# marbl/MHAP

Measured on AMD Instinct MI355X. Metric: overlaps/sec, higher is better.
Workload: dtype int64

## Files before the change

### mhap_amd/csrc/sketch_kernels.hip

```cpp
#include <cstdlib>
#include <cstring>

#include "kernels.hpp"
#include <algorithm>

namespace mhap {

constexpr int HASH_SEG = 4096;
constexpr int HASH_LUT_WORDS = 3 * 256;

void build_kmer_hash_luts(uint64_t* out) {
  const uint64_t c1 = 0x87c37b91114253d5ULL, c2 = 0x4cf5ad432745937fULL;
  const uint32_t d1 = 0xcc9e2d51U, d2 = 0x1b873593U;
  const char* acgt = "ACGT";
  for (int idx = 0; idx < 256; idx++) {
    uint64_t block = 0;
    for (int c = 0; c < 4; c++) block |= (uint64_t)(uint8_t)acgt[(idx >> (2 * c)) & 3] << (16 * c);
    uint64_t k1 = block * c1; k1 = rotl64(k1, 31); k1 *= c2;
    uint64_t k2 = block * c2; k2 = rotl64(k2, 33); k2 *= c1;
    uint32_t a = (uint32_t)block, b = (uint32_t)(block >> 32);
    a *= d1; a = rotl32(a, 15); a *= d2;
    b *= d1; b = rotl32(b, 15); b *= d2;
    out[idx] = k1; out[256 + idx] = k2; out[512 + idx] = (uint64_t)a | ((uint64_t)b << 32);
  }
// ... 1760 lines not shown
    return true;
  } else {
    const int waves_wg = (int)block.x / 64;
    const char* split_env = getenv("MHAP_MINHASH_SPLIT");
    const bool split_ok = !(split_env && atoi(split_env) == 0);
    const bool split = split_ok && waves_wg == 4 && n_weighted > 0 && n_weighted * 4 <= nblocks;
    const int nb_w = n_weighted < 0 ? nblocks : (int)std::min<int64_t>(nblocks, split ? n_weighted : (n_weighted + waves_wg - 1) / waves_wg);
    const int nb_u = n_unweighted < 0 ? nblocks : (int)std::min<int64_t>(nblocks, (n_unweighted + waves_wg - 1) / waves_wg);
    if (nb_w > 0)
      hipLaunchKernelGGL((minhash_kernel<MH_U, true, true>), dim3(nb_w), block, lds + 16, st_weighted, descs, nstrands, keys, wts, perm, info, store, luts, k, k2, H,
                         counter_w, out_rows, out_stride, out_status, status_stride, jump, jump_na, slist_w, counter + 5, qbuf_w, qcap, nullptr, split ? 1 : 0);
    char w1_path[160] = "none";
    if (nb_u > 0 && (classic || n_unweighted < 0 || waves_wg != 4)) {
      hipLaunchKernelGGL((minhash_kernel<MH_U, true, false>), dim3(nb_u), block, lds, st, descs, nstrands, keys, wts, perm, info, store, luts, k, k2, H,
                         counter_u, out_rows, out_stride, out_status, status_stride, jump, jump_na, slist, counter + 4, qbuf, qcap);
      if (witness) snprintf(w1_path, sizeof(w1_path), "classic");
    } else if (nb_u > 0) {
      W1Args a;
      a.descs = descs; a.keys = keys; a.store = store; a.luts = luts; a.info = info; a.slist = slist;
      a.n_tail = minhash_tail_strands(nblocks, n_unweighted); a.n_whole = n_unweighted - a.n_tail;
      a.rmax = max_nk > 0 ? (max_nk + 2047) >> 11 : 1;
      a.k = k; a.k2 = k2; a.H = H; a.counter = counter_u; a.stat = counter_u + 8;
      a.out_rows = out_rows; a.out_stride = out_stride; a.out_status = out_status; a.status_stride = status_stride;
      a.jump = jump_w1; a.unjump = unjump; a.jump_na = W1_JUMP_NA; a.qbuf = qbuf; a.qcap = qcap; a.merge = merge;
      {
        const char* e = getenv("MHAP_W1_STAGGER");
        const int stag = e ? atoi(e) : -1;
        a.stagger = stag >= 0 ? stag : 0;
      }
      const long long items = a.n_whole + a.n_tail * (long long)a.rmax;
      const int nb = (int)std::min<long long>(nblocks, (items + 3) / 4);
      const size_t lds1 = (size_t)H * 8 * 4 + lut_bytes;
      if (a.n_tail > 0) (void)hipMemsetAsync(merge, 0xFF, (size_t)a.n_tail * (size_t)H * 8, st);
      a.prof = nullptr;
      if (profmode) {
        static unsigned long long* dprof1 = nullptr;
        if (!dprof1) (void)hipMalloc(&dprof1, 8 * sizeof(unsigned long long));
        (void)hipMemsetAsync(dprof1, 0, 8 * sizeof(unsigned long long), st);
        a.prof = dprof1;
        static hipEvent_t pe0 = nullptr, pe1 = nullptr;
        if (!pe0) { (void)hipEventCreate(&pe0); (void)hipEventCreate(&pe1); }
        (void)hipEventRecord(pe0, st);
        if (qcap == BS_QCAP) hipLaunchKernelGGL((minhash_w1_kernel<true, true>), dim3(nb), dim3(256), lds1, st, a);
        else hipLaunchKernelGGL((minhash_w1_kernel<true, false>), dim3(nb), dim3(256), lds1, st, a);
        (void)hipEventRecord(pe1, st);
        unsigned long long hp[8];
        (void)hipMemcpyAsync(hp, dprof1, sizeof(hp), hipMemcpyDeviceToHost, st);
        (void)hipStreamSynchronize(st);
        const double tot = (double)hp[7];
        float pms = 0.f; (void)hipEventElapsedTime(&pms, pe0, pe1);
        fprintf(stderr, "[minhash w1 prof] launch %.3f ms, %d waves: mean shader clock %.0f MHz (wave-clocks / waves / time)\n", pms, nb * 4,
                pms > 0.f ? tot / ((double)nb * 4.0) / ((double)pms * 1e3) : 0.0);
        fprintf(stderr, "[minhash w1 prof] rows %llu (first-type %llu)  wave-clocks: total %.3g  key load+transpose %.1f%%  first-row slots %.1f%% (%.0f clocks/step)  "
                        "later-row slots %.1f%% (%.0f clocks/step)  drains %.1f%%  candidates/row %.0f\n", hp[4], hp[5], tot, 100.0 * hp[0] / tot, 100.0 * hp[1] / tot,
                hp[5] ? (double)hp[1] / ((double)hp[5] * H) : 0.0, 100.0 * hp[2] / tot, hp[4] > hp[5] ? (double)hp[2] / ((double)(hp[4] - hp[5]) * H) : 0.0,
                100.0 * hp[3] / tot, hp[4] ? (double)hp[6] / (double)hp[4] : 0.0);
      } else
        if (qcap == BS_QCAP) hipLaunchKernelGGL((minhash_w1_kernel<false, true>), dim3(nb), dim3(256), lds1, st, a);
        else hipLaunchKernelGGL((minhash_w1_kernel<false, false>), dim3(nb), dim3(256), lds1, st, a);
      if (a.n_tail > 0)
        hipLaunchKernelGGL(minhash_w1_finish_kernel, dim3((unsigned)((a.n_tail * (long long)H + 255) / 256)), dim3(256), 0, st, a);
      if (witness) snprintf(w1_path, sizeof(w1_path), "w1 n_whole %lld n_tail %lld rmax %d stagger %d", (long long)a.n_whole, (long long)a.n_tail, a.rmax, a.stagger);
    }
    if (witness)
      fprintf(stderr, "[minhash] strands %lld weight-1 %lld weighted %lld nblocks %d: weight-1 launch %s; weighted launch %s\n", (long long)nstrands,
              (long long)n_unweighted, (long long)n_weighted, nblocks, w1_path, nb_w > 0 ? (split ? "split" : "wave") : "none");
    return nb_w > 0;
  }
}


#ifdef MH_ORD_PROF
__device__ unsigned long long g_ord_prof[8];
#define ORD_TICK(k) do { __syncthreads(); if (threadIdx.x == 0) { const unsigned long long t_ = wall_clock64(); atomicAdd(&g_ord_prof[k], t_ - ord_t0); ord_t0 = t_; } } while (0)
#else
#define ORD_TICK(k) do { } while (0)
#endif
__device__ __forceinline__ uint32_t mm3_mul5c(uint32_t h) {
  uint32_t t;
  asm("v_lshl_add_u32 %0, %1, 2, %1" : "=v"(t) : "v"(h));
  return t + 0xe6546b64U;
}
constexpr uint32_t ORD_BUCKET_MAX = 32;
__device__ inline uint64_t okey(int32_t h, int pos) { return ((uint64_t)((uint32_t)h ^ 0x80000000u) << 32) | (uint32_t)pos; }

__global__ __launch_bounds__(ORD_THREADS) void ordered_kernel(const ReadDesc* __restrict__ descs, int64_t nstrands,
                                                              const int32_t* __restrict__ h32, const uint8_t* __restrict__ store,
                                                              const uint64_t* __restrict__ luts, int code_words, int stage_wide, int k2, int S, int cap,
                                                              int32_t* __restrict__ out_rows, int64_t out_stride,
                                                              int32_t* __restrict__ out_meta, int64_t meta_stride, int64_t first) {
  extern __shared__ __attribute__((aligned(16))) char smem[];
  uint32_t* hist = (uint32_t*)smem;
  uint32_t* part = hist + ORD_BINS;
  uint32_t* svars = part + ORD_THREADS;
  uint64_t* buf = (uint64_t*)(svars + 4);
  uint16_t* bstart = (uint16_t*)(buf + cap);
  uint32_t* stage = (uint32_t*)(bstart + ORD_BINS + 2);
  uint16_t* stage16 = (uint16_t*)stage;
  const size_t lut_off = ((size_t)ORD_BINS * 4 + (size_t)ORD_THREADS * 4 + 16 + (size_t)cap * 8 + (size_t)(ORD_BINS + 2) * 2 + (size_t)cap * (stage_wide ? 4 : 2) + 7) & ~(size_t)7;
  uint64_t* lut = (uint64_t*)(smem + lut_off);
  uint32_t* codes = (uint32_t*)(lut + 256);
  uint32_t& s_bin = svars[0]; uint32_t& s_below = svars[1]; uint32_t& s_cnt = svars[2]; uint32_t& s_fill = svars[3];
  const int64_t strand = first + (int64_t)blockIdx.x;
  if (strand >= nstrands) return;
#ifdef MH_ORD_PROF
  unsigned long long ord_t0 = wall_clock64();
#endif
  const ReadDesc rd = descs[strand >> 1];
  const int rcs = (int)(strand & 1);
  const int n = rd.length - k2 + 1;
  int32_t* meta = out_meta + strand * meta_stride;
  if (strand_skipped(rd, rcs) || n < 1) {
    if (threadIdx.x == 0) { meta[0] = 0; meta[1] = n; meta[2] = rd.length; }
    return;
  }
  const bool mat = (rd.flags & MHAP_RD_MAT) != 0;
  const int32_t* hp = h32 + rd.h2_off + (rcs ? rd.h2_stride : 0);
  if (!mat) {
    for (int i = threadIdx.x; i < 256; i += ORD_THREADS) lut[i] = luts[512 + i];
    const int ncw = (rd.length + 15) / 16 + 2;
    for (int wj = threadIdx.x; wj < ncw && wj < code_words; wj += ORD_THREADS) codes[wj] = strand_codes16(store + rd.base_off, rd.length, rcs, 16 * wj);
    __syncthreads();
  }
  ORD_TICK(0);
  auto hget = [&](int i) -> int32_t {
    if (mat) return hp[i];
    const uint32_t cw = codes_at(codes, i);
    uint32_t h = 0;
#pragma unroll
    for (int q = 0; q < 3; q++) {
      const uint64_t kk = lut[(cw >> (8 * q)) & 255u];
      h ^= (uint32_t)kk;         h = rotl32(h, 13); h = mm3_mul5c(h);
      h ^= (uint32_t)(kk >> 32); h = rotl32(h, 13); h = mm3_mul5c(h);
    }
    h ^= 24u;
    return (int32_t)fmix32(h);
  };
  const int K = S < n ? S : n;
  if (threadIdx.x == 0) { meta[0] = K; meta[1] = n; meta[2] = rd.length; }
  if (K <= 0) return;

  const double ksig = sqrt((double)K), csig = sqrt((double)cap);
  const double target = fmin((double)K + 7.0 * ksig, (double)cap - 5.0 * csig);
  if (n > cap && target >= (double)K + 3.0 * ksig) {
    const double quant = target / (double)n;
    const uint32_t cut_u = quant >= 1.0 ? 0xFFFFFFFFu : (uint32_t)(quant * 4294967296.0);
    const uint32_t cutbin = cut_u >> 21;
    for (uint32_t j = threadIdx.x; j < ORD_BINS; j += ORD_THREADS) hist[j] = 0;
    if (threadIdx.x == 0) { s_fill = 0; s_cnt = 0; }
    __syncthreads();
    const int lane = threadIdx.x & 63;
    for (int ib = 0; ib < n; ib += 8 * ORD_THREADS) {
      const int p0 = ib + 32 * (int)(threadIdx.x >> 2) + (int)(threadIdx.x & 3);
      int32_t hv[8];
      if (mat) {
#pragma unroll
        for (int u = 0; u < 8; u++) { const int i = p0 + 4 * u; hv[u] = i < n ? hp[i] : 0; }
      } else if (p0 < n) {
        const int d = p0 >> 4;
        const uint32_t sh = (uint32_t)(2 * (p0 & 15));
        const uint32_t w0 = codes[d], w1 = codes[d + 1], w2 = codes[d + 2], w3 = codes[d + 3];
        const uint32_t a[3] = {__builtin_amdgcn_alignbit(w1, w0, sh), __builtin_amdgcn_alignbit(w2, w1, sh), __builtin_amdgcn_alignbit(w3, w2, sh)};
        uint64_t g[10];
#pragma unroll
        for (int j = 0; j < 10; j++) g[j] = lut[(a[j >> 2] >> (8 * (j & 3))) & 255u];
#pragma unroll
        for (int u = 0; u < 8; u++) {
          uint32_t h = 0;
#pragma unroll
          for (int q = 0; q < 3; q++) {
            const uint64_t kk = g[u + q];
            h ^= (uint32_t)kk;         h = rotl32(h, 13); h = mm3_mul5c(h);
            h ^= (uint32_t)(kk >> 32); h = rotl32(h, 13); h = mm3_mul5c(h);
          }
          h ^= 24u;
          hv[u] = (int32_t)fmix32(h);
        }
      } else {
#pragma unroll
        for (int u = 0; u < 8; u++) hv[u] = 0;
      }
      unsigned long long bal[8];
      uint32_t total = 0;
#pragma unroll
      for (int u = 0; u < 8; u++) {
        bal[u] = __ballot(p0 + 4 * u < n && ((uint32_t)hv[u] ^ 0x80000000u) < cut_u);
        total += (uint32_t)__popcll(bal[u]);
      }
      if (total) {
        uint32_t base = 0;
        if (lane == 0) base = atomicAdd(&s_fill, total);
        base = (uint32_t)__builtin_amdgcn_readfirstlane((int)base);
#pragma unroll
        for (int u = 0; u < 8; u++) {
          if ((bal[u] >> lane) & 1ULL) {
            const uint32_t idx = base + __builtin_amdgcn_mbcnt_hi((uint32_t)(bal[u] >> 32), __builtin_amdgcn_mbcnt_lo((uint32_t)bal[u], 0u));
            if (idx < (uint32_t)cap) { if (stage_wide) stage[idx] = (uint32_t)(p0 + 4 * u); else stage16[idx] = (uint16_t)(p0 + 4 * u); }
            atomicAdd(&hist[((uint32_t)hv[u] ^ 0x80000000u) >> 21], 1u);
          }
          base += (uint32_t)__popcll(bal[u]);
        }
      }
    }
    __syncthreads();
    ORD_TICK(1);
    const uint32_t m = s_fill;
    bool ok = m >= (uint32_t)K && m <= (uint32_t)cap;
    if (ok) {
      const int per = ORD_BINS / ORD_THREADS;
      uint32_t loc = 0, mx = 0;
      for (int j = 0; j < per; j++) { const uint32_t c = hist[threadIdx.x * per + j]; loc += c; mx = c > mx ? c : mx; }
      uint32_t incl = loc;
#pragma unroll
      for (int off = 1; off < 64; off <<= 1) { const uint32_t v = __shfl_up(incl, off); if (lane >= off) incl += v; }
      if (lane == 63) part[threadIdx.x >> 6] = incl;
      if (mx > ORD_BUCKET_MAX) atomicMax(&s_cnt, mx);
      __syncthreads();
      for (unsigned w = 0; w < (threadIdx.x >> 6); w++) incl += part[w];
      uint32_t run = incl - loc;
      for (int j = 0; j < per; j++) { const uint32_t b = threadIdx.x * per + j; bstart[b] = (uint16_t)run; run += hist[b]; }
      ok = s_cnt == 0;
      __syncthreads();
    }
    ORD_TICK(2);
    if (ok) {
      for (uint32_t b = threadIdx.x; b <= cutbin; b += ORD_THREADS) hist[b] = 0;
      __syncthreads();
      for (uint32_t t0 = threadIdx.x; t0 < m; t0 += 4 * ORD_THREADS) {
        int ii[4]; uint64_t key[4]; uint32_t slot[4];
#pragma unroll
        for (int u = 0; u < 4; u++) { const uint32_t t = t0 + (uint32_t)u * ORD_THREADS; ii[u] = t < m ? (stage_wide ? (int)stage[t] : (int)stage16[t]) : 0; }
#pragma unroll
        for (int u = 0; u < 4; u++) key[u] = okey(hget(ii[u]), ii[u]);
#pragma unroll
        for (int u = 0; u < 4; u++) { const uint32_t b = (uint32_t)(key[u] >> 53); slot[u] = t0 + (uint32_t)u * ORD_THREADS < m ? (uint32_t)bstart[b] + atomicAdd(&hist[b], 1u) : 0xFFFFFFFFu; }
#pragma unroll
        for (int u = 0; u < 4; u++) if (slot[u] != 0xFFFFFFFFu) buf[slot[u]] = key[u];
      }
      __syncthreads();
      ORD_TICK(3);
      int32_t* orow = out_rows + strand * out_stride;
      for (uint32_t t0 = threadIdx.x; t0 < m; t0 += 2 * ORD_THREADS) {
        uint64_t key[2]; uint32_t s0[2], c[2], rank[2] = {0u, 0u};
#pragma unroll
        for (int u = 0; u < 2; u++) {
          const uint32_t t = t0 + (uint32_t)u * ORD_THREADS;
          key[u] = buf[t < m ? t : t0];
          const uint32_t b = (uint32_t)(key[u] >> 53);
          s0[u] = bstart[b]; c[u] = t < m ? hist[b] : 0u;
        }
        const uint32_t cmax = c[0] > c[1] ? c[0] : c[1];
        for (uint32_t q = 0; q < cmax; q += 4) {
          uint64_t o[2][4];
#pragma unroll
          for (int u = 0; u < 2; u++)
#pragma unroll
            for (int x = 0; x < 4; x++) o[u][x] = buf[s0[u] + q + (uint32_t)x < (uint32_t)cap ? s0[u] + q + (uint32_t)x : s0[u]];
#pragma unroll
          for (int u = 0; u < 2; u++)
#pragma unroll
            for (int x = 0; x < 4; x++) rank[u] += (q + (uint32_t)x < c[u] && o[u][x] < key[u]) ? 1u : 0u;
        }
#pragma unroll
        for (int u = 0; u < 2; u++) {
          const uint32_t j = s0[u] + rank[u];
          if (t0 + (uint32_t)u * ORD_THREADS < m && j < (uint32_t)K) { orow[2 * j] = (int32_t)((uint32_t)(key[u] >> 32) ^ 0x80000000u); orow[2 * j + 1] = (int32_t)(uint32_t)key[u]; }
        }
      }
      ORD_TICK(5);
#ifdef MH_ORD_PROF
      if (threadIdx.x == 0) atomicAdd(&g_ord_prof[7], 1ULL);
#endif
      return;
    }
    __syncthreads();
  }

  uint64_t bound = ~0ULL;
  bool buckets = false;
  uint32_t bk_bin = 0, bk_total = 0;
  if (threadIdx.x == 0) s_fill = 0;
  if (n > cap) {
    const int shifts[6] = {53, 42, 32, 21, 10, 0};
    const int widths[6] = {11, 11, 10, 11, 11, 10};
    uint64_t prefix = 0;
    uint64_t prefmask = 0;
    uint32_t below = 0;
    for (int lv = 0; lv < 6; lv++) {
      const int sh = shifts[lv];
      const uint32_t nb = 1u << widths[lv];
      for (uint32_t j = threadIdx.x; j < ORD_BINS; j += ORD_THREADS) hist[j] = 0;
      __syncthreads();
      for (int i0 = threadIdx.x; i0 < n; i0 += 8 * ORD_THREADS) {
        int32_t hv[8];
#pragma unroll
        for (int u = 0; u < 8; u++) { const int i = i0 + u * ORD_THREADS; hv[u] = i < n ? hget(i) : 0; }
#pragma unroll
        for (int u = 0; u < 8; u++) {
          const int i = i0 + u * ORD_THREADS;
          const uint64_t key = okey(hv[u], i);
          if (i < n && (key & prefmask) == prefix) atomicAdd(&hist[(uint32_t)(key >> sh) & (nb - 1)], 1u);
        }
      }
      __syncthreads();
      const uint32_t target = (uint32_t)(K - 1) - below;
      const int per = ORD_BINS / ORD_THREADS;
      uint32_t loc = 0;
      for (int j = 0; j < per; j++) loc += hist[threadIdx.x * per + j];
      uint32_t incl = loc;
#pragma unroll
      for (int off = 1; off < 64; off <<= 1) {
        const uint32_t v = __shfl_up(incl, off);
        if ((threadIdx.x & 63) >= (unsigned)off) incl += v;
      }
      if ((threadIdx.x & 63) == 63) part[threadIdx.x >> 6] = incl;
      __syncthreads();
      for (unsigned w = 0; w < (threadIdx.x >> 6); w++) incl += part[w];
      const uint32_t excl = incl - loc;
      if (target >= excl && target < incl) {
        uint32_t run = excl;
        for (int j = 0; j < per; j++) {
          const uint32_t c = hist[threadIdx.x * per + j];
          if (target < run + c) { s_bin = threadIdx.x * per + j; s_below = run; s_cnt = c; break; }
          run += c;
        }
      }
      __syncthreads();
      const uint32_t bin = s_bin, binbelow = s_below, bincnt = s_cnt;
      __syncthreads();
      below += binbelow;
      prefix |= (uint64_t)bin << sh;
      prefmask |= (uint64_t)(nb - 1) << sh;
      bound = prefix | (sh > 0 ? ((1ULL << sh) - 1) : 0ULL);
      if (below + bincnt <= (uint32_t)cap) {
        if (lv == 0) {
          uint32_t run = excl, mx = 0;
          for (int j = 0; j < per; j++) {
            const uint32_t b = threadIdx.x * per + j, c = hist[b];
            if (b <= bin) { bstart[b] = (uint16_t)run; mx = c > mx ? c : mx; }
            run += c;
          }
          if (mx > ORD_BUCKET_MAX) atomicMax(&s_fill, mx);
          __syncthreads();
          buckets = s_fill == 0;
          bk_bin = bin; bk_total = below + bincnt;
          __syncthreads();
          if (threadIdx.x == 0) s_fill = 0;
        }
        break;
      }
    }
  }
  if (buckets) {
    for (uint32_t b = threadIdx.x; b <= bk_bin; b += ORD_THREADS) hist[b] = 0;
    __syncthreads();
    for (int i0 = threadIdx.x; i0 < n; i0 += 8 * ORD_THREADS) {
      int32_t hv[8];
#pragma unroll
      for (int u = 0; u < 8; u++) { const int i = i0 + u * ORD_THREADS; hv[u] = i < n ? hget(i) : 0; }
#pragma unroll
      for (int u = 0; u < 8; u++) {
        const int i = i0 + u * ORD_THREADS;
        const uint64_t key = okey(hv[u], i);
        const uint32_t b = (uint32_t)(key >> 53);
        if (i < n && b <= bk_bin) buf[(uint32_t)bstart[b] + atomicAdd(&hist[b], 1u)] = key;
      }
    }
    __syncthreads();
    int32_t* orow = out_rows + strand * out_stride;
    for (uint32_t t = threadIdx.x; t < bk_total; t += ORD_THREADS) {
      const uint64_t key = buf[t];
      const uint32_t b = (uint32_t)(key >> 53), s0 = bstart[b], c = hist[b];
      uint32_t rank = 0;
      for (uint32_t q = 0; q < c; q += 4) {
        uint64_t o[4];
#pragma unroll
        for (int x = 0; x < 4; x++) o[x] = buf[s0 + q + (uint32_t)x < (uint32_t)cap ? s0 + q + (uint32_t)x : s0];
#pragma unroll
        for (int x = 0; x < 4; x++) rank += (q + (uint32_t)x < c && o[x] < key) ? 1u : 0u;
      }
      const uint32_t j = s0 + rank;
      if (j < (uint32_t)K) { orow[2 * j] = (int32_t)((uint32_t)(key >> 32) ^ 0x80000000u); orow[2 * j + 1] = (int32_t)(uint32_t)key; }
    }
    return;
  }
  __syncthreads();
  for (int i = threadIdx.x; i < n; i += ORD_THREADS) {
    const uint64_t key = okey(hget(i), i);
    if (key <= bound) { uint32_t slot = atomicAdd(&s_fill, 1u); if (slot < (uint32_t)cap) buf[slot] = key; }
  }
  __syncthreads();
  const uint32_t m = s_fill < (uint32_t)cap ? s_fill : (uint32_t)cap;
  uint32_t np2 = 1;
  while (np2 < m) np2 <<= 1;
  for (uint32_t j = m + threadIdx.x; j < np2; j += ORD_THREADS) buf[j] = ~0ULL;
  __syncthreads();
  for (uint32_t size = 2; size <= np2; size <<= 1) {
    for (uint32_t stride = size >> 1; stride > 0; stride >>= 1) {
      for (uint32_t t = threadIdx.x; t < (np2 >> 1); t += ORD_THREADS) {
        const uint32_t lo = 2 * t - (t & (stride - 1));
        const uint32_t hi = lo + stride;
        const bool up = ((lo & size) == 0);
        const uint64_t a = buf[lo], b = buf[hi];
        if ((a > b) == up) { buf[lo] = b; buf[hi] = a; }
      }
      __syncthreads();
    }
  }
  int32_t* orow = out_rows + strand * out_stride;
  for (int j = threadIdx.x; j < K; j += ORD_THREADS) {
    const uint64_t key = buf[j];
    orow[2 * j] = (int32_t)((uint32_t)(key >> 32) ^ 0x80000000u);
    orow[2 * j + 1] = (int32_t)(uint32_t)key;
  }
}

#ifndef MH_ORD_PAD
#define MH_ORD_PAD 0
#endif
size_t ordered_lds_bytes(int cap, int code_words, int stage_wide) {
  return (size_t)ORD_BINS * 4 + (size_t)ORD_THREADS * 4 + 16 + (size_t)cap * 8 + (size_t)(ORD_BINS + 2) * 2 + (size_t)cap * (stage_wide ? 4 : 2) +
         (code_words > 0 ? (size_t)256 * 8 + (size_t)code_words * 4 : 0) + 8 + MH_ORD_PAD;
}

__global__ void fix_status_kernel(int32_t* __restrict__ meta, int64_t nreads) {
  const int64_t i = (int64_t)blockIdx.x * blockDim.x + threadIdx.x;
  if (i >= nreads) return;
  const int32_t fs = meta[(2 * i) * META_W + 3];
  if (fs != 0 && meta[(2 * i + 1) * META_W + 3] == 0) meta[(2 * i + 1) * META_W + 3] = fs;
}

void launch_fix_status(hipStream_t st, int32_t* meta, int64_t nreads) {
  if (nreads <= 0) return;
  hipLaunchKernelGGL(fix_status_kernel, dim3((unsigned)((nreads + 255) / 256)), dim3(256), 0, st, meta, nreads);
}

void launch_ordered(hipStream_t st, const ReadDesc* descs, int64_t nstrands, int max_len_codes, int max_len, const int32_t* h32,
                    const uint8_t* store, const uint64_t* luts, int k2, int S, int cap, int32_t* out_rows, int64_t out_stride,
                    int32_t* out_meta, int64_t meta_stride, int64_t first, int64_t count) {
  if (count < 0 || first + count > nstrands) count = nstrands - first;
  if (nstrands <= 0 || count <= 0) return;
  const int code_words = max_len_codes > 0 ? (max_len_codes + 15) / 16 + 4 : 0;
  const int stage_wide = max_len - k2 + 1 > 65535 ? 1 : 0;
  hipLaunchKernelGGL(ordered_kernel, dim3((unsigned)count), dim3(ORD_THREADS), ordered_lds_bytes(cap, code_words, stage_wide), st, descs, nstrands, h32,
                     store, luts, code_words, stage_wide, k2, S, cap, out_rows, out_stride, out_meta, meta_stride, first);
#ifdef MH_ORD_PROF
  (void)hipStreamSynchronize(st);
  unsigned long long hp[8];
  (void)hipMemcpyFromSymbol(hp, HIP_SYMBOL(g_ord_prof), sizeof(hp));
  fprintf(stderr, "[ordered prof] cap %d lds %zu strands(one-pass) %llu  100MHz ticks/strand: stage %.1f pass1 %.1f scan %.1f fill %.1f isort %.1f out %.1f\n", cap,
          ordered_lds_bytes(cap, code_words, stage_wide), hp[7], (double)hp[0] / hp[7], (double)hp[1] / hp[7], (double)hp[2] / hp[7], (double)hp[3] / hp[7],
          (double)hp[4] / hp[7], (double)hp[5] / hp[7]);
  unsigned long long z[8] = {0, 0, 0, 0, 0, 0, 0, 0};
  (void)hipMemcpyToSymbol(HIP_SYMBOL(g_ord_prof), z, sizeof(z));
#endif
}

}
```

Baseline: 445,000.

## Process both strands of a read in one double-width ordered-sketch workgroup

The ordered kernel now launches one 512-thread workgroup per read instead of one 256-thread block per strand. Each half handles one strand from a single shared copy of the forward 2-bit codes, and the reverse complement is built on the fly with a bit-reverse trick. The histogram bin count is sized from cap with an adaptive shift, and bucket offsets are packed into the histogram words to save LDS. This cuts the duplicated code staging and per-block overhead, but adds LDS per workgroup (two buffers), which may reduce occupancy and makes the fallback path more complex.

```diff
diff --git a/mhap_amd/csrc/sketch_kernels.hip b/mhap_amd/csrc/sketch_kernels.hip
--- a/mhap_amd/csrc/sketch_kernels.hip
+++ b/mhap_amd/csrc/sketch_kernels.hip
@@ -1866,50 +1866,81 @@
   return t + 0xe6546b64U;
 }
 constexpr uint32_t ORD_BUCKET_MAX = 32;
+constexpr int ORD_WG = 2 * ORD_THREADS;
+constexpr int ORD_PADW = 4;
 __device__ inline uint64_t okey(int32_t h, int pos) { return ((uint64_t)((uint32_t)h ^ 0x80000000u) << 32) | (uint32_t)pos; }
-
-__global__ __launch_bounds__(ORD_THREADS) void ordered_kernel(const ReadDesc* __restrict__ descs, int64_t nstrands,
-                                                              const int32_t* __restrict__ h32, const uint8_t* __restrict__ store,
-                                                              const uint64_t* __restrict__ luts, int code_words, int stage_wide, int k2, int S, int cap,
-                                                              int32_t* __restrict__ out_rows, int64_t out_stride,
-                                                              int32_t* __restrict__ out_meta, int64_t meta_stride, int64_t first) {
+__device__ __forceinline__ uint32_t rc_codes16(uint32_t x) {
+  x = __builtin_bitreverse32(x);
+  return ~(((x >> 1) & 0x55555555u) | ((x & 0x55555555u) << 1));
+}
+__host__ __device__ inline int ord_bins(int cap) { return cap / 4 < 256 ? 256 : (cap / 4 > ORD_BINS ? ORD_BINS : cap / 4); }
+struct OrdLds {
+  size_t half, uni, buf, lut, codes, total;
+  __host__ __device__ OrdLds(int cap, int code_words, int stage_wide) {
+    half = ((size_t)ord_bins(cap) * 4 + (size_t)cap * (stage_wide ? 4 : 2) + 7) & ~(size_t)7;
+    const size_t exact = (size_t)ORD_BINS * 4 + (((size_t)(ORD_BINS + 2) * 2 + 7) & ~(size_t)7);
+    uni = 96;
+    buf = uni + (2 * half > exact ? 2 * half : exact);
+    lut = buf + (size_t)cap * 16;
+    codes = lut + (code_words > 0 ? (size_t)256 * 8 : 0);
+    total = codes + (code_words > 0 ? (size_t)(ORD_PADW + code_words) * 4 : 0);
+  }
+};
+
+__global__ __launch_bounds__(ORD_WG) void ordered_kernel(const ReadDesc* __restrict__ descs, int64_t nreads,
+                                                         const int32_t* __restrict__ h32, const uint8_t* __restrict__ store,
+                                                         const uint64_t* __restrict__ luts, int code_words, int stage_wide, int k2, int S, int cap,
+                                                         int32_t* __restrict__ out_rows, int64_t out_stride,
+                                                         int32_t* __restrict__ out_meta, int64_t meta_stride, int64_t first_read) {
   extern __shared__ __attribute__((aligned(16))) char smem[];
-  uint32_t* hist = (uint32_t*)smem;
-  uint32_t* part = hist + ORD_BINS;
-  uint32_t* svars = part + ORD_THREADS;
-  uint64_t* buf = (uint64_t*)(svars + 4);
-  uint16_t* bstart = (uint16_t*)(buf + cap);
-  uint32_t* stage = (uint32_t*)(bstart + ORD_BINS + 2);
-  uint16_t* stage16 = (uint16_t*)stage;
-  const size_t lut_off = ((size_t)ORD_BINS * 4 + (size_t)ORD_THREADS * 4 + 16 + (size_t)cap * 8 + (size_t)(ORD_BINS + 2) * 2 + (size_t)cap * (stage_wide ? 4 : 2) + 7) & ~(size_t)7;
-  uint64_t* lut = (uint64_t*)(smem + lut_off);
-  uint32_t* codes = (uint32_t*)(lut + 256);
-  uint32_t& s_bin = svars[0]; uint32_t& s_below = svars[1]; uint32_t& s_cnt = svars[2]; uint32_t& s_fill = svars[3];
-  const int64_t strand = first + (int64_t)blockIdx.x;
-  if (strand >= nstrands) return;
+  const OrdLds L(cap, code_words, stage_wide);
+  uint32_t* svars = (uint32_t*)smem;
+  uint32_t* part = svars + 16;
+  uint64_t* lut = (uint64_t*)(smem + L.lut);
+  uint32_t* cf = (uint32_t*)(smem + L.codes);
+  const int64_t read = first_read + (int64_t)blockIdx.x;
+  if (read >= nreads) return;
 #ifdef MH_ORD_PROF
   unsigned long long ord_t0 = wall_clock64();
 #endif
-  const ReadDesc rd = descs[strand >> 1];
-  const int rcs = (int)(strand & 1);
-  const int n = rd.length - k2 + 1;
-  int32_t* meta = out_meta + strand * meta_stride;
-  if (strand_skipped(rd, rcs) || n < 1) {
-    if (threadIdx.x == 0) { meta[0] = 0; meta[1] = n; meta[2] = rd.length; }
-    return;
-  }
+  const ReadDesc rd = descs[read];
+  const int Lr = rd.length;
+  const int n = Lr - k2 + 1;
+  const int K = S < n ? S : n;
+  const int hs = (int)(threadIdx.x >> 8);
+  const uint32_t tl = threadIdx.x & (ORD_THREADS - 1);
+  const int lane = threadIdx.x & 63;
+  const bool act0 = !strand_skipped(rd, 0) && n >= 1 && K > 0;
+  const bool act1 = !strand_skipped(rd, 1) && n >= 1 && K > 0;
+  if (tl == 0) {
+    int32_t* meta = out_meta + (2 * read + hs) * meta_stride;
+    meta[0] = (strand_skipped(rd, hs) || n < 1) ? 0 : K; meta[1] = n; meta[2] = Lr;
+  }
+  if (!act0 && !act1) return;
   const bool mat = (rd.flags & MHAP_RD_MAT) != 0;
-  const int32_t* hp = h32 + rd.h2_off + (rcs ? rd.h2_stride : 0);
   if (!mat) {
-    for (int i = threadIdx.x; i < 256; i += ORD_THREADS) lut[i] = luts[512 + i];
-    const int ncw = (rd.length + 15) / 16 + 2;
-    for (int wj = threadIdx.x; wj < ncw && wj < code_words; wj += ORD_THREADS) codes[wj] = strand_codes16(store + rd.base_off, rd.length, rcs, 16 * wj);
+    const uint32_t* W = (const uint32_t*)(store + rd.base_off);
+    const int nd = (Lr + 15) >> 4;
+    const int ncw = min(nd + 2, code_words);
+    if (threadIdx.x < 256) lut[threadIdx.x] = luts[512 + threadIdx.x];
+    if (threadIdx.x < ORD_PADW) cf[threadIdx.x] = 0u;
+    uint32_t v[2];
+#pragma unroll
+    for (int u = 0; u < 2; u++) { const int w = (int)threadIdx.x + u * ORD_WG; v[u] = w < nd ? W[w] : 0u; }
+#pragma unroll
+    for (int u = 0; u < 2; u++) { const int w = (int)threadIdx.x + u * ORD_WG; if (w < ncw) cf[ORD_PADW + w] = v[u]; }
+    for (int w = (int)threadIdx.x + 2 * ORD_WG; w < ncw; w += ORD_WG) cf[ORD_PADW + w] = w < nd ? W[w] : 0u;
     __syncthreads();
   }
   ORD_TICK(0);
-  auto hget = [&](int i) -> int32_t {
-    if (mat) return hp[i];
-    const uint32_t cw = codes_at(codes, i);
+  auto cwin = [&](int s, int p) -> uint32_t {
+    const int q = (s ? Lr - 16 - p : p) + 16 * ORD_PADW;
+    const uint32_t x = __builtin_amdgcn_alignbit(cf[(q >> 4) + 1], cf[q >> 4], (uint32_t)(2 * (q & 15)));
+    return s ? rc_codes16(x) : x;
+  };
+  auto hget = [&](int s, int i) -> int32_t {
+    if (mat) return h32[rd.h2_off + (s ? rd.h2_stride : 0) + i];
+    const uint32_t cw = cwin(s, i);
     uint32_t h = 0;
 #pragma unroll
     for (int q = 0; q < 3; q++) {
@@ -1920,118 +1951,138 @@
     h ^= 24u;
     return (int32_t)fmix32(h);
   };
-  const int K = S < n ? S : n;
-  if (threadIdx.x == 0) { meta[0] = K; meta[1] = n; meta[2] = rd.length; }
-  if (K <= 0) return;
-
+
+  bool need0 = act0, need1 = act1;
   const double ksig = sqrt((double)K), csig = sqrt((double)cap);
   const double target = fmin((double)K + 7.0 * ksig, (double)cap - 5.0 * csig);
   if (n > cap && target >= (double)K + 3.0 * ksig) {
     const double quant = target / (double)n;
     const uint32_t cut_u = quant >= 1.0 ? 0xFFFFFFFFu : (uint32_t)(quant * 4294967296.0);
-    const uint32_t cutbin = cut_u >> 21;
-    for (uint32_t j = threadIdx.x; j < ORD_BINS; j += ORD_THREADS) hist[j] = 0;
-    if (threadIdx.x == 0) { s_fill = 0; s_cnt = 0; }
-    __syncthreads();
-    const int lane = threadIdx.x & 63;
-    for (int ib = 0; ib < n; ib += 8 * ORD_THREADS) {
-      const int p0 = ib + 32 * (int)(threadIdx.x >> 2) + (int)(threadIdx.x & 3);
-      int32_t hv[8];
-      if (mat) {
-#pragma unroll
-        for (int u = 0; u < 8; u++) { const int i = p0 + 4 * u; hv[u] = i < n ? hp[i] : 0; }
-      } else if (p0 < n) {
-        const int d = p0 >> 4;
-        const uint32_t sh = (uint32_t)(2 * (p0 & 15));
-        const uint32_t w0 = codes[d], w1 = codes[d + 1], w2 = codes[d + 2], w3 = codes[d + 3];
-        const uint32_t a[3] = {__builtin_amdgcn_alignbit(w1, w0, sh), __builtin_amdgcn_alignbit(w2, w1, sh), __builtin_amdgcn_alignbit(w3, w2, sh)};
-        uint64_t g[10];
-#pragma unroll
-        for (int j = 0; j < 10; j++) g[j] = lut[(a[j >> 2] >> (8 * (j & 3))) & 255u];
+    const int nbins = ord_bins(cap);
+    const int lgb = 31 - __builtin_clz((uint32_t)nbins);
+    const int hb = cut_u ? 31 - __builtin_clz(cut_u) : -1;
+    const int bsh = hb + 1 - lgb > 0 ? hb + 1 - lgb : 0;
+    const bool act = hs ? act1 : act0;
+    uint32_t* hist = (uint32_t*)(smem + L.uni + (size_t)hs * L.half);
+    uint32_t* stage = hist + nbins;
+    uint16_t* stage16 = (uint16_t*)stage;
+    uint64_t* buf = (uint64_t*)(smem + L.buf) + (size_t)hs * cap;
+    uint32_t& s_fill = svars[hs];
+    uint32_t& s_cnt = svars[2 + hs];
+    for (uint32_t j = tl; j < (uint32_t)nbins; j += ORD_THREADS) hist[j] = 0;
+    if (tl == 0) { s_fill = 0; s_cnt = 0; }
+    __syncthreads();
+    if (act) {
+      const int32_t* hp = h32 + rd.h2_off + (hs ? rd.h2_stride : 0);
+      for (int ib = 0; ib < n; ib += 8 * ORD_THREADS) {
+        const int p0 = ib + 32 * (int)(tl >> 2) + (int)(tl & 3);
+        int32_t hv[8];
+        if (mat) {
+#pragma unroll
+          for (int u = 0; u < 8; u++) { const int i = p0 + 4 * u; hv[u] = i < n ? hp[i] : 0; }
+        } else if (p0 < n) {
+          const int q = (hs ? Lr - 48 - p0 : p0) + 16 * ORD_PADW;
+          const int d = q >> 4;
+          const uint32_t sh = (uint32_t)(2 * (q & 15));
+          const uint32_t w0 = cf[d], w1 = cf[d + 1], w2 = cf[d + 2], w3 = cf[d + 3];
+          const uint32_t b0 = __builtin_amdgcn_alignbit(w1, w0, sh), b1 = __builtin_amdgcn_alignbit(w2, w1, sh), b2 = __builtin_amdgcn_alignbit(w3, w2, sh);
+          const uint32_t a[3] = {hs ? rc_codes16(b2) : b0, hs ? rc_codes16(b1) : b1, hs ? rc_codes16(b0) : b2};
+          uint64_t g[10];
+#pragma unroll
+          for (int j = 0; j < 10; j++) g[j] = lut[(a[j >> 2] >> (8 * (j & 3))) & 255u];
+#pragma unroll
+          for (int u = 0; u < 8; u++) {
+            uint32_t h = 0;
+#pragma unroll
+            for (int qq = 0; qq < 3; qq++) {
+              const uint64_t kk = g[u + qq];
+              h ^= (uint32_t)kk;         h = rotl32(h, 13); h = mm3_mul5c(h);
+              h ^= (uint32_t)(kk >> 32); h = rotl32(h, 13); h = mm3_mul5c(h);
+            }
+            h ^= 24u;
+            hv[u] = (int32_t)fmix32(h);
+          }
+        } else {
+#pragma unroll
+          for (int u = 0; u < 8; u++) hv[u] = 0;
+        }
+        unsigned long long bal[8];
+        uint32_t total = 0;
 #pragma unroll
         for (int u = 0; u < 8; u++) {
-          uint32_t h = 0;
-#pragma unroll
-          for (int q = 0; q < 3; q++) {
-            const uint64_t kk = g[u + q];
-            h ^= (uint32_t)kk;         h = rotl32(h, 13); h = mm3_mul5c(h);
-            h ^= (uint32_t)(kk >> 32); h = rotl32(h, 13); h = mm3_mul5c(h);
+          bal[u] = __ballot(p0 + 4 * u < n && ((uint32_t)hv[u] ^ 0x80000000u) < cut_u);
+          total += (uint32_t)__popcll(bal[u]);
+        }
+        if (total) {
+          uint32_t base = 0;
+          if (lane == 0) base = atomicAdd(&s_fill, total);
+          base = (uint32_t)__builtin_amdgcn_readfirstlane((int)base);
+#pragma unroll
+          for (int u = 0; u < 8; u++) {
+            if ((bal[u] >> lane) & 1ULL) {
+              const uint32_t idx = base + __builtin_amdgcn_mbcnt_hi((uint32_t)(bal[u] >> 32), __builtin_amdgcn_mbcnt_lo((uint32_t)bal[u], 0u));
+              if (idx < (uint32_t)cap) { if (stage_wide) stage[idx] = (uint32_t)(p0 + 4 * u); else stage16[idx] = (uint16_t)(p0 + 4 * u); }
+              atomicAdd(&hist[(((uint32_t)hv[u] ^ 0x80000000u) >> bsh) & (uint32_t)(nbins - 1)], 1u);
+            }
+            base += (uint32_t)__popcll(bal[u]);
           }
-          h ^= 24u;
-          hv[u] = (int32_t)fmix32(h);
-        }
-      } else {
-#pragma unroll
-        for (int u = 0; u < 8; u++) hv[u] = 0;
-      }
-      unsigned long long bal[8];
-      uint32_t total = 0;
-#pragma unroll
-      for (int u = 0; u < 8; u++) {
-        bal[u] = __ballot(p0 + 4 * u < n && ((uint32_t)hv[u] ^ 0x80000000u) < cut_u);
-        total += (uint32_t)__popcll(bal[u]);
-      }
-      if (total) {
-        uint32_t base = 0;
-        if (lane == 0) base = atomicAdd(&s_fill, total);
-        base = (uint32_t)__builtin_amdgcn_readfirstlane((int)base);
-#pragma unroll
-        for (int u = 0; u < 8; u++) {
-          if ((bal[u] >> lane) & 1ULL) {
-            const uint32_t idx = base + __builtin_amdgcn_mbcnt_hi((uint32_t)(bal[u] >> 32), __builtin_amdgcn_mbcnt_lo((uint32_t)bal[u], 0u));
-            if (idx < (uint32_t)cap) { if (stage_wide) stage[idx] = (uint32_t)(p0 + 4 * u); else stage16[idx] = (uint16_t)(p0 + 4 * u); }
-            atomicAdd(&hist[((uint32_t)hv[u] ^ 0x80000000u) >> 21], 1u);
-          }
-          base += (uint32_t)__popcll(bal[u]);
         }
       }
     }
     __syncthreads();
     ORD_TICK(1);
     const uint32_t m = s_fill;
-    bool ok = m >= (uint32_t)K && m <= (uint32_t)cap;
+    bool ok = act && m >= (uint32_t)K && m <= (uint32_t)cap;
+    const int per = nbins / ORD_THREADS;
+    uint32_t loc = 0, incl = 0;
     if (ok) {
-      const int per = ORD_BINS / ORD_THREADS;
-      uint32_t loc = 0, mx = 0;
-      for (int j = 0; j < per; j++) { const uint32_t c = hist[threadIdx.x * per + j]; loc += c; mx = c > mx ? c : mx; }
-      uint32_t incl = loc;
+      uint32_t mx = 0;
+      for (int j = 0; j < per; j++) { const uint32_t c = hist[tl * per + j]; loc += c; mx = c > mx ? c : mx; }
+      incl = loc;
 #pragma unroll
       for (int off = 1; off < 64; off <<= 1) { const uint32_t v = __shfl_up(incl, off); if (lane >= off) incl += v; }
       if (lane == 63) part[threadIdx.x >> 6] = incl;
       if (mx > ORD_BUCKET_MAX) atomicMax(&s_cnt, mx);
-      __syncthreads();
-      for (unsigned w = 0; w < (threadIdx.x >> 6); w++) incl += part[w];
+    }
+    __syncthreads();
+    ok = ok && s_cnt == 0;
+    if (ok) {
+      for (uint32_t w = 0; w < (tl >> 6); w++) incl += part[(threadIdx.x >> 8) * 4 + w];
       uint32_t run = incl - loc;
-      for (int j = 0; j < per; j++) { const uint32_t b = threadIdx.x * per + j; bstart[b] = (uint16_t)run; run += hist[b]; }
-      ok = s_cnt == 0;
-      __syncthreads();
-    }
+      for (int j = 0; j < per; j++) { const uint32_t b = tl * per + j, c = hist[b]; hist[b] = run << 16; run += c; }
+    }
+    __syncthreads();
     ORD_TICK(2);
     if (ok) {
-      for (uint32_t b = threadIdx.x; b <= cutbin; b += ORD_THREADS) hist[b] = 0;
-      __syncthreads();
-      for (uint32_t t0 = threadIdx.x; t0 < m; t0 += 4 * ORD_THREADS) {
+      for (uint32_t t0 = tl; t0 < m; t0 += 4 * ORD_THREADS) {
         int ii[4]; uint64_t key[4]; uint32_t slot[4];
 #pragma unroll
         for (int u = 0; u < 4; u++) { const uint32_t t = t0 + (uint32_t)u * ORD_THREADS; ii[u] = t < m ? (stage_wide ? (int)stage[t] : (int)stage16[t]) : 0; }
 #pragma unroll
-        for (int u = 0; u < 4; u++) key[u] = okey(hget(ii[u]), ii[u]);
-#pragma unroll
-        for (int u = 0; u < 4; u++) { const uint32_t b = (uint32_t)(key[u] >> 53); slot[u] = t0 + (uint32_t)u * ORD_THREADS < m ? (uint32_t)bstart[b] + atomicAdd(&hist[b], 1u) : 0xFFFFFFFFu; }
+        for (int u = 0; u < 4; u++) key[u] = okey(hget(hs, ii[u]), ii[u]);
+#pragma unroll
+        for (int u = 0; u < 4; u++) {
+          const uint32_t b = (uint32_t)(key[u] >> (32 + bsh)) & (uint32_t)(nbins - 1);
+          uint32_t w = 0xFFFFFFFFu;
+          if (t0 + (uint32_t)u * ORD_THREADS < m) { w = atomicAdd(&hist[b], 1u); w = (w >> 16) + (w & 0xFFFFu); }
+          slot[u] = w;
+        }
 #pragma unroll
         for (int u = 0; u < 4; u++) if (slot[u] != 0xFFFFFFFFu) buf[slot[u]] = key[u];
       }
-      __syncthreads();
-      ORD_TICK(3);
-      int32_t* orow = out_rows + strand * out_stride;
-      for (uint32_t t0 = threadIdx.x; t0 < m; t0 += 2 * ORD_THREADS) {
+    }
+    __syncthreads();
+    ORD_TICK(3);
+    if (ok) {
+      int32_t* orow = out_rows + (2 * read + hs) * out_stride;
+      for (uint32_t t0 = tl; t0 < m; t0 += 2 * ORD_THREADS) {
         uint64_t key[2]; uint32_t s0[2], c[2], rank[2] = {0u, 0u};
 #pragma unroll
         for (int u = 0; u < 2; u++) {
           const uint32_t t = t0 + (uint32_t)u * ORD_THREADS;
           key[u] = buf[t < m ? t : t0];
-          const uint32_t b = (uint32_t)(key[u] >> 53);
-          s0[u] = bstart[b]; c[u] = t < m ? hist[b] : 0u;
+          const uint32_t hw = hist[(uint32_t)(key[u] >> (32 + bsh)) & (uint32_t)(nbins - 1)];
+          s0[u] = hw >> 16; c[u] = t < m ? (hw & 0xFFFFu) : 0u;
         }
         const uint32_t cmax = c[0] > c[1] ? c[0] : c[1];
         for (uint32_t q = 0; q < cmax; q += 4) {
@@ -2051,161 +2102,168 @@
           if (t0 + (uint32_t)u * ORD_THREADS < m && j < (uint32_t)K) { orow[2 * j] = (int32_t)((uint32_t)(key[u] >> 32) ^ 0x80000000u); orow[2 * j + 1] = (int32_t)(uint32_t)key[u]; }
         }
       }
-      ORD_TICK(5);
+    }
+    ORD_TICK(5);
 #ifdef MH_ORD_PROF
-      if (threadIdx.x == 0) atomicAdd(&g_ord_prof[7], 1ULL);
+    if (threadIdx.x == 0) atomicAdd(&g_ord_prof[7], 1ULL);
 #endif
-      return;
-    }
-    __syncthreads();
-  }
-
-  uint64_t bound = ~0ULL;
-  bool buckets = false;
-  uint32_t bk_bin = 0, bk_total = 0;
-  if (threadIdx.x == 0) s_fill = 0;
-  if (n > cap) {
-    const int shifts[6] = {53, 42, 32, 21, 10, 0};
-    const int widths[6] = {11, 11, 10, 11, 11, 10};
-    uint64_t prefix = 0;
-    uint64_t prefmask = 0;
-    uint32_t below = 0;
-    for (int lv = 0; lv < 6; lv++) {
-      const int sh = shifts[lv];
-      const uint32_t nb = 1u << widths[lv];
-      for (uint32_t j = threadIdx.x; j < ORD_BINS; j += ORD_THREADS) hist[j] = 0;
-      __syncthreads();
-      for (int i0 = threadIdx.x; i0 < n; i0 += 8 * ORD_THREADS) {
-        int32_t hv[8];
-#pragma unroll
-        for (int u = 0; u < 8; u++) { const int i = i0 + u * ORD_THREADS; hv[u] = i < n ? hget(i) : 0; }
-#pragma unroll
-        for (int u = 0; u < 8; u++) {
-          const int i = i0 + u * ORD_THREADS;
-          const uint64_t key = okey(hv[u], i);
-          if (i < n && (key & prefmask) == prefix) atomicAdd(&hist[(uint32_t)(key >> sh) & (nb - 1)], 1u);
+    const uint32_t m0 = svars[0], m1 = svars[1];
+    need0 = act0 && !(m0 >= (uint32_t)K && m0 <= (uint32_t)cap && svars[2] == 0);
+    need1 = act1 && !(m1 >= (uint32_t)K && m1 <= (uint32_t)cap && svars[3] == 0);
+    if (!need0 && !need1) return;
+    __syncthreads();
+  }
+
+  uint32_t* hist = (uint32_t*)(smem + L.uni);
+  uint16_t* bstart = (uint16_t*)(smem + L.uni + (size_t)ORD_BINS * 4);
+  uint64_t* buf = (uint64_t*)(smem + L.buf);
+  uint32_t& s_bin = svars[4]; uint32_t& s_below = svars[5]; uint32_t& s_cnt = svars[6]; uint32_t& s_fill = svars[7];
+  for (int s = 0; s < 2; s++) {
+    if (!(s ? need1 : need0)) continue;
+    uint64_t bound = ~0ULL;
+    bool buckets = false;
+    uint32_t bk_bin = 0, bk_total = 0;
+    __syncthreads();
+    if (threadIdx.x == 0) s_fill = 0;
+    if (n > cap) {
+      const int shifts[6] = {53, 42, 32, 21, 10, 0};
+      const int widths[6] = {11, 11, 10, 11, 11, 10};
+      uint64_t prefix = 0;
+      uint64_t prefmask = 0;
+      uint32_t below = 0;
+      for (int lv = 0; lv < 6; lv++) {
+        const int sh = shifts[lv];
+        const uint32_t nb = 1u << widths[lv];
+        for (uint32_t j = threadIdx.x; j < ORD_BINS; j += ORD_WG) hist[j] = 0;
+        __syncthreads();
+        for (int i0 = threadIdx.x; i0 < n; i0 += 8 * ORD_WG) {
+          int32_t hv[8];
+#pragma unroll
+          for (int u = 0; u < 8; u++) { const int i = i0 + u * ORD_WG; hv[u] = i < n ? hget(s, i) : 0; }
+#pragma unroll
+          for (int u = 0; u < 8; u++) {
+            const int i = i0 + u * ORD_WG;
+            const uint64_t key = okey(hv[u], i);
+            if (i < n && (key & prefmask) == prefix) atomicAdd(&hist[(uint32_t)(key >> sh) & (nb - 1)], 1u);
+          }
         }
-      }
-      __syncthreads();
-      const uint32_t target = (uint32_t)(K - 1) - below;
-      const int per = ORD_BINS / ORD_THREADS;
-      uint32_t loc = 0;
-      for (int j = 0; j < per; j++) loc += hist[threadIdx.x * per + j];
-      uint32_t incl = loc;
-#pragma unroll
-      for (int off = 1; off < 64; off <<= 1) {
-        const uint32_t v = __shfl_up(incl, off);
-        if ((threadIdx.x & 63) >= (unsigned)off) incl += v;
-      }
-      if ((threadIdx.x & 63) == 63) part[threadIdx.x >> 6] = incl;
-      __syncthreads();
-      for (unsigned w = 0; w < (threadIdx.x >> 6); w++) incl += part[w];
-      const uint32_t excl = incl - loc;
-      if (target >= excl && target < incl) {
-        uint32_t run = excl;
-        for (int j = 0; j < per; j++) {
-          const uint32_t c = hist[threadIdx.x * per + j];
-          if (target < run + c) { s_bin = threadIdx.x * per + j; s_below = run; s_cnt = c; break; }
-          run += c;
+        __syncthreads();
+        const uint32_t target = (uint32_t)(K - 1) - below;
+        const int per = ORD_BINS / ORD_WG;
+        uint32_t loc = 0;
+        for (int j = 0; j < per; j++) loc += hist[threadIdx.x * per + j];
+        uint32_t incl = loc;
+#pragma unroll
+        for (int off = 1; off < 64; off <<= 1) {
+          const uint32_t v = __shfl_up(incl, off);
+          if ((threadIdx.x & 63) >= (unsigned)off) incl += v;
         }
-      }
-      __syncthreads();
-      const uint32_t bin = s_bin, binbelow = s_below, bincnt = s_cnt;
-      __syncthreads();
-      below += binbelow;
-      prefix |= (uint64_t)bin << sh;
-      prefmask |= (uint64_t)(nb - 1) << sh;
-      bound = prefix | (sh > 0 ? ((1ULL << sh) - 1) : 0ULL);
-      if (below + bincnt <= (uint32_t)cap) {
-        if (lv == 0) {
-          uint32_t run = excl, mx = 0;
+        if ((threadIdx.x & 63) == 63) part[threadIdx.x >> 6] = incl;
+        __syncthreads();
+        for (unsigned w = 0; w < (threadIdx.x >> 6); w++) incl += part[w];
+        const uint32_t excl = incl - loc;
+        if (target >= excl && target < incl) {
+          uint32_t run = excl;
           for (int j = 0; j < per; j++) {
-            const uint32_t b = threadIdx.x * per + j, c = hist[b];
-            if (b <= bin) { bstart[b] = (uint16_t)run; mx = c > mx ? c : mx; }
+            const uint32_t c = hist[threadIdx.x * per + j];
+            if (target < run + c) { s_bin = threadIdx.x * per + j; s_below = run; s_cnt = c; break; }
             run += c;
           }
-          if (mx > ORD_BUCKET_MAX) atomicMax(&s_fill, mx);
-          __syncthreads();
-          buckets = s_fill == 0;
-          bk_bin = bin; bk_total = below + bincnt;
-          __syncthreads();
-          if (threadIdx.x == 0) s_fill = 0;
         }
-        break;
-      }
-    }
-  }
-  if (buckets) {
-    for (uint32_t b = threadIdx.x; b <= bk_bin; b += ORD_THREADS) hist[b] = 0;
-    __syncthreads();
-    for (int i0 = threadIdx.x; i0 < n; i0 += 8 * ORD_THREADS) {
-      int32_t hv[8];
-#pragma unroll
-      for (int u = 0; u < 8; u++) { const int i = i0 + u * ORD_THREADS; hv[u] = i < n ? hget(i) : 0; }
-#pragma unroll
-      for (int u = 0; u < 8; u++) {
-        const int i = i0 + u * ORD_THREADS;
-        const uint64_t key = okey(hv[u], i);
-        const uint32_t b = (uint32_t)(key >> 53);
-        if (i < n && b <= bk_bin) buf[(uint32_t)bstart[b] + atomicAdd(&hist[b], 1u)] = key;
-      }
-    }
-    __syncthreads();
-    int32_t* orow = out_rows + strand * out_stride;
-    for (uint32_t t = threadIdx.x; t < bk_total; t += ORD_THREADS) {
-      const uint64_t key = buf[t];
-      const uint32_t b = (uint32_t)(key >> 53), s0 = bstart[b], c = hist[b];
-      uint32_t rank = 0;
-      for (uint32_t q = 0; q < c; q += 4) {
-        uint64_t o[4];
-#pragma unroll
-        for (int x = 0; x < 4; x++) o[x] = buf[s0 + q + (uint32_t)x < (uint32_t)cap ? s0 + q + (uint32_t)x : s0];
-#pragma unroll
-        for (int x = 0; x < 4; x++) rank += (q + (uint32_t)x < c && o[x] < key) ? 1u : 0u;
-      }
-      const uint32_t j = s0 + rank;
-      if (j < (uint32_t)K) { orow[2 * j] = (int32_t)((uint32_t)(key >> 32) ^ 0x80000000u); orow[2 * j + 1] = (int32_t)(uint32_t)key; }
-    }
-    return;
-  }
-  __syncthreads();
-  for (int i = threadIdx.x; i < n; i += ORD_THREADS) {
-    const uint64_t key = okey(hget(i), i);
-    if (key <= bound) { uint32_t slot = atomicAdd(&s_fill, 1u); if (slot < (uint32_t)cap) buf[slot] = key; }
-  }
-  __syncthreads();
-  const uint32_t m = s_fill < (uint32_t)cap ? s_fill : (uint32_t)cap;
-  uint32_t np2 = 1;
-  while (np2 < m) np2 <<= 1;
-  for (uint32_t j = m + threadIdx.x; j < np2; j += ORD_THREADS) buf[j] = ~0ULL;
-  __syncthreads();
-  for (uint32_t size = 2; size <= np2; size <<= 1) {
-    for (uint32_t stride = size >> 1; stride > 0; stride >>= 1) {
-      for (uint32_t t = threadIdx.x; t < (np2 >> 1); t += ORD_THREADS) {
-        const uint32_t lo = 2 * t - (t & (stride - 1));
-        const uint32_t hi = lo + stride;
-        const bool up = ((lo & size) == 0);
-        const uint64_t a = buf[lo], b = buf[hi];
-        if ((a > b) == up) { buf[lo] = b; buf[hi] = a; }
-      }
+        __syncthreads();
+        const uint32_t bin = s_bin, binbelow = s_below, bincnt = s_cnt;
+        __syncthreads();
+        below += binbelow;
+        prefix |= (uint64_t)bin << sh;
+        prefmask |= (uint64_t)(nb - 1) << sh;
+        bound = prefix | (sh > 0 ? ((1ULL << sh) - 1) : 0ULL);
+        if (below + bincnt <= (uint32_t)cap) {
+          if (lv == 0) {
+            uint32_t run = excl, mx = 0;
+            for (int j = 0; j < per; j++) {
+              const uint32_t b = threadIdx.x * per + j, c = hist[b];
+              if (b <= bin) { bstart[b] = (uint16_t)run; mx = c > mx ? c : mx; }
+              run += c;
+            }
+            if (mx > ORD_BUCKET_MAX) atomicMax(&s_fill, mx);
+            __syncthreads();
+            buckets = s_fill == 0;
+            bk_bin = bin; bk_total = below + bincnt;
+            __syncthreads();
+            if (threadIdx.x == 0) s_fill = 0;
+          }
+          break;
+        }
+      }
+    }
+    int32_t* orow = out_rows + (2 * read + s) * out_stride;
+    if (buckets) {
+      for (uint32_t b = threadIdx.x; b <= bk_bin; b += ORD_WG) hist[b] = 0;
       __syncthreads();
-    }
-  }
-  int32_t* orow = out_rows + strand * out_stride;
-  for (int j = threadIdx.x; j < K; j += ORD_THREADS) {
-    const uint64_t key = buf[j];
-    orow[2 * j] = (int32_t)((uint32_t)(key >> 32) ^ 0x80000000u);
-    orow[2 * j + 1] = (int32_t)(uint32_t)key;
+      for (int i0 = threadIdx.x; i0 < n; i0 += 8 * ORD_WG) {
+        int32_t hv[8];
+#pragma unroll
+        for (int u = 0; u < 8; u++) { const int i = i0 + u * ORD_WG; hv[u] = i < n ? hget(s, i) : 0; }
+#pragma unroll
+        for (int u = 0; u < 8; u++) {
+          const int i = i0 + u * ORD_WG;
+          const uint64_t key = okey(hv[u], i);
+          const uint32_t b = (uint32_t)(key >> 53);
+          if (i < n && b <= bk_bin) buf[(uint32_t)bstart[b] + atomicAdd(&hist[b], 1u)] = key;
+        }
+      }
+      __syncthreads();
+      for (uint32_t t = threadIdx.x; t < bk_total; t += ORD_WG) {
+        const uint64_t key = buf[t];
+        const uint32_t b = (uint32_t)(key >> 53), s0 = bstart[b], c = hist[b];
+        uint32_t rank = 0;
+        for (uint32_t q = 0; q < c; q += 4) {
+          uint64_t o[4];
+#pragma unroll
+          for (int x = 0; x < 4; x++) o[x] = buf[s0 + q + (uint32_t)x < (uint32_t)cap ? s0 + q + (uint32_t)x : s0];
+#pragma unroll
+          for (int x = 0; x < 4; x++) rank += (q + (uint32_t)x < c && o[x] < key) ? 1u : 0u;
+        }
+        const uint32_t j = s0 + rank;
+        if (j < (uint32_t)K) { orow[2 * j] = (int32_t)((uint32_t)(key >> 32) ^ 0x80000000u); orow[2 * j + 1] = (int32_t)(uint32_t)key; }
+      }
+      continue;
+    }
+    __syncthreads();
+    for (int i = threadIdx.x; i < n; i += ORD_WG) {
+      const uint64_t key = okey(hget(s, i), i);
+      if (key <= bound) { uint32_t slot = atomicAdd(&s_fill, 1u); if (slot < (uint32_t)cap) buf[slot] = key; }
+    }
+    __syncthreads();
+    const uint32_t m = s_fill < (uint32_t)cap ? s_fill : (uint32_t)cap;
+    uint32_t np2 = 1;
+    while (np2 < m) np2 <<= 1;
+    for (uint32_t j = m + threadIdx.x; j < np2; j += ORD_WG) buf[j] = ~0ULL;
+    __syncthreads();
+    for (uint32_t size = 2; size <= np2; size <<= 1) {
+      for (uint32_t stride = size >> 1; stride > 0; stride >>= 1) {
+        for (uint32_t t = threadIdx.x; t < (np2 >> 1); t += ORD_WG) {
+          const uint32_t lo = 2 * t - (t & (stride - 1));
+          const uint32_t hi = lo + stride;
+          const bool up = ((lo & size) == 0);
+          const uint64_t a = buf[lo], b = buf[hi];
+          if ((a > b) == up) { buf[lo] = b; buf[hi] = a; }
+        }
+        __syncthreads();
+      }
+    }
+    for (int j = threadIdx.x; j < K; j += ORD_WG) {
+      const uint64_t key = buf[j];
+      orow[2 * j] = (int32_t)((uint32_t)(key >> 32) ^ 0x80000000u);
+      orow[2 * j + 1] = (int32_t)(uint32_t)key;
+    }
   }
 }
 
 #ifndef MH_ORD_PAD
 #define MH_ORD_PAD 0
 #endif
-size_t ordered_lds_bytes(int cap, int code_words, int stage_wide) {
-  return (size_t)ORD_BINS * 4 + (size_t)ORD_THREADS * 4 + 16 + (size_t)cap * 8 + (size_t)(ORD_BINS + 2) * 2 + (size_t)cap * (stage_wide ? 4 : 2) +
-         (code_words > 0 ? (size_t)256 * 8 + (size_t)code_words * 4 : 0) + 8 + MH_ORD_PAD;
-}
+size_t ordered_lds_bytes(int cap, int code_words, int stage_wide) { return OrdLds(cap, code_words, stage_wide).total + MH_ORD_PAD; }
 
 __global__ void fix_status_kernel(int32_t* __restrict__ meta, int64_t nreads) {
   const int64_t i = (int64_t)blockIdx.x * blockDim.x + threadIdx.x;
@@ -2224,15 +2282,17 @@
                     int32_t* out_meta, int64_t meta_stride, int64_t first, int64_t count) {
   if (count < 0 || first + count > nstrands) count = nstrands - first;
   if (nstrands <= 0 || count <= 0) return;
+  const int64_t nreads = nstrands / 2, r0 = first / 2, r1 = std::min<int64_t>(nreads, (first + count + 1) / 2);
+  if (r1 <= r0) return;
   const int code_words = max_len_codes > 0 ? (max_len_codes + 15) / 16 + 4 : 0;
   const int stage_wide = max_len - k2 + 1 > 65535 ? 1 : 0;
-  hipLaunchKernelGGL(ordered_kernel, dim3((unsigned)count), dim3(ORD_THREADS), ordered_lds_bytes(cap, code_words, stage_wide), st, descs, nstrands, h32,
-                     store, luts, code_words, stage_wide, k2, S, cap, out_rows, out_stride, out_meta, meta_stride, first);
+  hipLaunchKernelGGL(ordered_kernel, dim3((unsigned)(r1 - r0)), dim3(ORD_WG), ordered_lds_bytes(cap, code_words, stage_wide), st, descs, nreads, h32,
+                     store, luts, code_words, stage_wide, k2, S, cap, out_rows, out_stride, out_meta, meta_stride, r0);
 #ifdef MH_ORD_PROF
   (void)hipStreamSynchronize(st);
   unsigned long long hp[8];
   (void)hipMemcpyFromSymbol(hp, HIP_SYMBOL(g_ord_prof), sizeof(hp));
-  fprintf(stderr, "[ordered prof] cap %d lds %zu strands(one-pass) %llu  100MHz ticks/strand: stage %.1f pass1 %.1f scan %.1f fill %.1f isort %.1f out %.1f\n", cap,
+  fprintf(stderr, "[ordered prof] cap %d lds %zu reads(one-pass) %llu  100MHz ticks/read: stage %.1f pass1 %.1f scan %.1f fill %.1f isort %.1f out %.1f\n", cap,
           ordered_lds_bytes(cap, code_words, stage_wide), hp[7], (double)hp[0] / hp[7], (double)hp[1] / hp[7], (double)hp[2] / hp[7], (double)hp[3] / hp[7],
           (double)hp[4] / hp[7], (double)hp[5] / hp[7]);
   unsigned long long z[8] = {0, 0, 0, 0, 0, 0, 0, 0};
```

Result: no change. 444,400, median of 3 (-0.1%).
